# eric-downes/tianshou_marl

Hardware: AMD Instinct MI355X
Metric: env-steps/sec (n_env x n_agent) incl. PPO update, simple_spread N=3 (higher is better)
Workload: dtype f32; 1 GPU; simple_spread_v3 N=3 shared PPO, num_envs=1024 per GPU, obs 18, A=5, T=25, MLP 64-64; minibatch=4096, repeat=1, dispatch=per_agent, parallelism=env-shard x1

## Files before the change

### tianshou_marl_amd/csrc/mlp_tile.h

```cpp
#pragma once
#include "common.h"

namespace {

constexpr int R = 16;
constexpr int NT = 256;
constexpr int kMaxJ = 4;

struct Dims {
    int D, A;
    int Kp1;
    int nJ;
    int ld1;
};

__host__ __device__ constexpr Dims dims_const(int D, int A) {
    Dims d{};
    d.D = D; d.A = A; d.Kp1 = (D + 3) / 4 * 4; d.nJ = (D + 15) / 16; d.ld1 = 16 * ((D + 15) / 16) + 2;
    return d;
}

template <int H>
struct Lay {
    static constexpr int ldh = H + 2;
    static constexpr int ld2 = 2 * H + 2;
    static constexpr int ldo = 18;
    int W1, W2a, W2c, W3a, W3c, B1, B2, B3a, B3c, X, H1, H2, OUT, D3, D2, D1, total;
    __host__ __device__ Lay(const Dims &d, bool bwd) {
        int o = 0;
        W1 = o; o += 2 * H * d.ld1;
        W2a = o; o += H * ldh;
        W2c = o; o += H * ldh;
        W3a = o; o += 16 * ldh;
        W3c = o; o += H;
        B1 = o; o += 2 * H;
        B2 = o; o += 2 * H;
        B3a = o; o += 16;
        B3c = o; o += 2;
        o = (o + 3) & ~3;
        X = o; o += R * d.ld1;
        H1 = o; o += R * ld2;
        H2 = o; o += R * ld2;
        OUT = o; o += R * ldo;
        D3 = o; o += bwd ? R * ldo : 0;
        D2 = o; o += bwd ? R * ld2 : 0;
        D1 = o; o += bwd ? R * ld2 : 0;
        total = o;
    }
};

__device__ __forceinline__ f4 mfma(float a, float b, f4 c) {
    return __builtin_amdgcn_mfma_f32_16x16x4f32(a, b, c, 0, 0, 0);
}

template <int N>
__device__ __forceinline__ float fmaf_chain_ahead(const float *h, const float *w) {
    constexpr int Q = 8;
    static_assert(N % (2 * Q) == 0, "pairs of whole groups");
    float h0[Q], w0[Q], h1[Q], w1[Q], s = 0.f;
    int off = 0;
    auto pin = [&]() { asm volatile("" : "+v"(s), "+v"(off)); };
#pragma unroll
    for (int p = 0; p < Q; ++p) { h0[p] = h[p]; w0[p] = w[p]; }
#pragma unroll
    for (int j0 = 0; j0 < N; j0 += 2 * Q) {
        pin();
#pragma unroll
        for (int p = 0; p < Q; ++p) { h1[p] = h[off + j0 + Q + p]; w1[p] = w[off + j0 + Q + p]; }
#pragma unroll
        for (int p = 0; p < Q; ++p) s = fmaf(h0[p], w0[p], s);
        pin();
        if (j0 + 2 * Q < N) {
#pragma unroll
            for (int p = 0; p < Q; ++p) { h0[p] = h[off + j0 + 2 * Q + p]; w0[p] = w[off + j0 + 2 * Q + p]; }
        }
#pragma unroll
        for (int p = 0; p < Q; ++p) s = fmaf(h1[p], w1[p], s);
    }
    return s;
}

template <int H>
struct POff {
    int aW1, ab1, aW2, ab2, aW3, ab3, cW1, cb1, cW2, cb2, cW3, cb3, total;
    __host__ __device__ POff(int D, int A) {
        int o = 0;
        aW1 = o; o += H * D; ab1 = o; o += H; aW2 = o; o += H * H; ab2 = o; o += H; aW3 = o; o += A * H; ab3 = o; o += A;
        cW1 = o; o += H * D; cb1 = o; o += H; cW2 = o; o += H * H; cb2 = o; o += H; cW3 = o; o += H; cb3 = o; o += 1;
        total = o;
    }
};

template <int H>
__device__ void stage_weights(float *lds, const Lay<H> &ly, const Dims &d, const float *__restrict__ P, int tid_in = -1) {
    const POff<H> po(d.D, d.A);
    const int tid = tid_in < 0 ? (int)threadIdx.x : tid_in;
    constexpr int U = 12;
    for (int e0 = tid; e0 < 2 * H * d.ld1; e0 += U * NT) {
        float v[U];
#pragma unroll
        for (int u = 0; u < U; ++u) {
            const int e = e0 + u * NT;
            const int row = e / d.ld1, c = e - row * d.ld1;
            v[u] = 0.f;
            if (e < 2 * H * d.ld1 && c < d.D) v[u] = row < H ? P[po.aW1 + row * d.D + c] : P[po.cW1 + (row - H) * d.D + c];
        }
#pragma unroll
        for (int u = 0; u < U; ++u)
            if (e0 + u * NT < 2 * H * d.ld1) lds[ly.W1 + e0 + u * NT] = v[u];
    }
    for (int e0 = tid; e0 < H * ly.ldh; e0 += U * NT) {
        float va[U], vc[U];
#pragma unroll
        for (int u = 0; u < U; ++u) {
            const int e = e0 + u * NT;
            const int row = e / ly.ldh, c = e - row * ly.ldh;
            const bool on = e < H * ly.ldh && c < H;
            va[u] = on ? P[po.aW2 + row * H + c] : 0.f;
            vc[u] = on ? P[po.cW2 + row * H + c] : 0.f;
        }
#pragma unroll
        for (int u = 0; u < U; ++u) {
            const int e = e0 + u * NT;
            if (e < H * ly.ldh) { lds[ly.W2a + e] = va[u]; lds[ly.W2c + e] = vc[u]; }
        }
    }
    {
        constexpr int N3 = (16 * Lay<H>::ldh + NT - 1) / NT;
        float v3[N3], vv[5];
#pragma unroll
        for (int u = 0; u < N3; ++u) {
            const int e = tid + u * NT, row = e / ly.ldh, c = e - row * ly.ldh;
            v3[u] = (e < 16 * ly.ldh && row < d.A && c < H) ? P[po.aW3 + row * H + c] : 0.f;
        }
        const int e5 = tid < H ? tid : 0;
        vv[0] = P[po.cW3 + e5]; vv[1] = P[po.ab1 + e5]; vv[2] = P[po.cb1 + e5]; vv[3] = P[po.ab2 + e5]; vv[4] = P[po.cb2 + e5];
#pragma unroll
        for (int u = 0; u < N3; ++u) {
            const int e = tid + u * NT;
            if (e < 16 * ly.ldh) lds[ly.W3a + e] = v3[u];
        }
        if (tid < H) {
            lds[ly.W3c + tid] = vv[0]; lds[ly.B1 + tid] = vv[1]; lds[ly.B1 + H + tid] = vv[2]; lds[ly.B2 + tid] = vv[3];
            lds[ly.B2 + H + tid] = vv[4];
        }
    }
    if (tid < 16) lds[ly.B3a + tid] = tid < d.A ? P[po.ab3 + tid] : 0.f;
    if (tid == 0) lds[ly.B3c] = P[po.cb3];
}

constexpr int kStageChunk = 4 * 256;
__host__ __device__ inline int image_f4_padded(int x_floats) {
    return ((x_floats / 4) + kStageChunk - 1) / kStageChunk * kStageChunk;
}

template <int H>
__device__ __forceinline__ void stage_image(float *lds, const Lay<H> &ly, const float *__restrict__ img) {
    const int n4p = image_f4_padded(ly.X);
    const int wave_base = (threadIdx.x >> 6) * 64;
    for (int e = 0; e < n4p; e += NT) {
        __builtin_amdgcn_global_load_lds(
            (const __attribute__((address_space(1))) void *)(img + (size_t)(e + threadIdx.x) * 4),
            (__attribute__((address_space(3))) void *)(lds + (size_t)(e + wave_base) * 4), 16, 0, 0);
    }
}

template <int H>
__device__ __forceinline__ void tile_forward(float *lds, const Lay<H> &ly, const Dims &d) {
    const int lane = threadIdx.x & 63, w = threadIdx.x >> 6;
    const int r16 = lane & 15, kq = lane >> 4;
    {
        f4 acc_a = {0.f, 0.f, 0.f, 0.f}, acc_c = {0.f, 0.f, 0.f, 0.f};
        const float *xa = lds + ly.X + r16 * d.ld1 + kq;
        const float *wa = lds + ly.W1 + (16 * w + r16) * d.ld1 + kq;
        const float *wc = lds + ly.W1 + (H + 16 * w + r16) * d.ld1 + kq;
        for (int k0 = 0; k0 < d.Kp1; k0 += 4) {
            const float a = xa[k0];
            acc_a = mfma(a, wa[k0], acc_a);
            acc_c = mfma(a, wc[k0], acc_c);
        }
        const int col = 16 * w + r16;
        const float ba = lds[ly.B1 + col], bc = lds[ly.B1 + H + col];
#pragma unroll
        for (int r = 0; r < 4; ++r) {
            const int row = kq * 4 + r;
            lds[ly.H1 + row * ly.ld2 + col] = fmaxf(acc_a[r] + ba, 0.f);
            lds[ly.H1 + row * ly.ld2 + H + col] = fmaxf(acc_c[r] + bc, 0.f);
        }
    }
    __syncthreads();
    {
        f4 acc_a = {0.f, 0.f, 0.f, 0.f}, acc_c = {0.f, 0.f, 0.f, 0.f};
        const float *ha = lds + ly.H1 + r16 * ly.ld2 + kq;
        const float *hc = ha + H;
        const float *wa = lds + ly.W2a + (16 * w + r16) * ly.ldh + kq;
        const float *wc = lds + ly.W2c + (16 * w + r16) * ly.ldh + kq;
#pragma unroll
        for (int k0 = 0; k0 < H; k0 += 4) {
            acc_a = mfma(ha[k0], wa[k0], acc_a);
            acc_c = mfma(hc[k0], wc[k0], acc_c);
        }
        const int col = 16 * w + r16;
        const float ba = lds[ly.B2 + col], bc = lds[ly.B2 + H + col];
#pragma unroll
        for (int r = 0; r < 4; ++r) {
            const int row = kq * 4 + r;
            lds[ly.H2 + row * ly.ld2 + col] = fmaxf(acc_a[r] + ba, 0.f);
            lds[ly.H2 + row * ly.ld2 + H + col] = fmaxf(acc_c[r] + bc, 0.f);
        }
    }
    __syncthreads();
    if (w == 0) {
        f4 acc = {0.f, 0.f, 0.f, 0.f};
        const float *ha = lds + ly.H2 + r16 * ly.ld2 + kq;
        const float *wa = lds + ly.W3a + r16 * ly.ldh + kq;
#pragma unroll
        for (int k0 = 0; k0 < H; k0 += 4) acc = mfma(ha[k0], wa[k0], acc);
        const float b = lds[ly.B3a + r16];
#pragma unroll
        for (int r = 0; r < 4; ++r) lds[ly.OUT + (kq * 4 + r) * ly.ldo + r16] = acc[r] + b;
    } else if (w == 1 && lane < R) {
        const float *hc = lds + ly.H2 + lane * ly.ld2 + H;
        float s = 0.f;
        for (int j = 0; j < H; ++j) s = fmaf(hc[j], lds[ly.W3c + j], s);
        lds[ly.OUT + lane * ly.ldo + 16] = s + lds[ly.B3c];
    }
    __syncthreads();
}

template <int H>
__device__ __forceinline__ void tile_forward_split(float *lds, const Lay<H> &ly, const Dims &d) {
    const int lane = threadIdx.x & 63, w8 = threadIdx.x >> 6, net = w8 >> 2, w = w8 & 3;
    const int r16 = lane & 15, kq = lane >> 4;
    const int col = 16 * w + r16;
    {
        f4 acc = {0.f, 0.f, 0.f, 0.f};
        const float *xa = lds + ly.X + r16 * d.ld1 + kq;
        const float *wp = lds + ly.W1 + (net * H + col) * d.ld1 + kq;
        for (int k0 = 0; k0 < d.Kp1; k0 += 4) acc = mfma(xa[k0], wp[k0], acc);
        const float b = lds[ly.B1 + net * H + col];
#pragma unroll
        for (int r = 0; r < 4; ++r) lds[ly.H1 + (kq * 4 + r) * ly.ld2 + net * H + col] = fmaxf(acc[r] + b, 0.f);
    }
    __syncthreads();
    {
        f4 acc = {0.f, 0.f, 0.f, 0.f};
        const float *ha = lds + ly.H1 + r16 * ly.ld2 + net * H + kq;
        const float *wp = lds + (net ? ly.W2c : ly.W2a) + col * ly.ldh + kq;
#pragma unroll
        for (int k0 = 0; k0 < H; k0 += 4) acc = mfma(ha[k0], wp[k0], acc);
        const float b = lds[ly.B2 + net * H + col];
#pragma unroll
        for (int r = 0; r < 4; ++r) lds[ly.H2 + (kq * 4 + r) * ly.ld2 + net * H + col] = fmaxf(acc[r] + b, 0.f);
    }
    __syncthreads();
    if (w8 == 0) {
        f4 acc = {0.f, 0.f, 0.f, 0.f};
        const float *ha = lds + ly.H2 + r16 * ly.ld2 + kq;
        const float *wa = lds + ly.W3a + r16 * ly.ldh + kq;
#pragma unroll
        for (int k0 = 0; k0 < H; k0 += 4) acc = mfma(ha[k0], wa[k0], acc);
        const float b = lds[ly.B3a + r16];
#pragma unroll
        for (int r = 0; r < 4; ++r) lds[ly.OUT + (kq * 4 + r) * ly.ldo + r16] = acc[r] + b;
    } else if (w8 == 5 && lane < R) {
        const float *hc = lds + ly.H2 + lane * ly.ld2 + H;
        float s = 0.f;
        for (int j = 0; j < H; ++j) s = fmaf(hc[j], lds[ly.W3c + j], s);
        lds[ly.OUT + lane * ly.ldo + 16] = s + lds[ly.B3c];
    }
    __syncthreads();
}

constexpr int kXRegs = (R * (16 * kMaxJ + 2) + NT - 1) / NT;

template <int HAS_PERM = -1>
__device__ __forceinline__ void prefetch_tile_ids_load(int64_t (&id)[kXRegs + 1], const Dims &d, const int64_t *__restrict__ perm,
                                                       int64_t first, int64_t row0, int64_t M) {
    const int64_t ir = row0 + (threadIdx.x >> 4);
    if (HAS_PERM == 1 || (HAS_PERM == -1 && perm)) {
#pragma unroll
        for (int it = 0; it < kXRegs; ++it) {
            const int e = threadIdx.x + it * NT, r = e / d.ld1;
            const int64_t i = row0 + r;
            id[it] = perm[(e < R * d.ld1 && i < M) ? i : row0];
        }
        id[kXRegs] = perm[ir < M ? ir : row0];
    } else {
#pragma unroll
        for (int it = 0; it < kXRegs; ++it) id[it] = first + row0 + (threadIdx.x + it * NT) / d.ld1;
        id[kXRegs] = first + ir;
    }
}
__device__ __forceinline__ int64_t prefetch_tile_ids_done(int64_t (&xs)[kXRegs], const int64_t (&id)[kXRegs + 1], const Dims &d,
                                                          int64_t row0, int64_t M) {
#pragma unroll
    for (int it = 0; it < kXRegs; ++it) {
        const int e = threadIdx.x + it * NT, r = e / d.ld1, c = e - r * d.ld1;
        xs[it] = (e < R * d.ld1 && c < d.D && row0 + r < M) ? id[it] * d.D + c : -1;
    }
    return row0 + (threadIdx.x >> 4) < M ? id[kXRegs] : -1;
}
__device__ __forceinline__ int64_t prefetch_tile_ids_done_nb(int64_t (&xs)[kXRegs], unsigned &ok, const int64_t (&id)[kXRegs + 1],
                                                             const Dims &d, int64_t row0, int64_t M) {
    ok = 0;
#pragma unroll
    for (int it = 0; it < kXRegs; ++it) {
        const int e = threadIdx.x + it * NT, r = e / d.ld1, c = e - r * d.ld1;
        xs[it] = id[it] * d.D + (c < d.D ? c : 0);
        ok |= (unsigned)(e < R * d.ld1 && c < d.D && row0 + r < M) << it;
    }
    return row0 + (threadIdx.x >> 4) < M ? id[kXRegs] : -1;
}
__device__ __forceinline__ void prefetch_tile_vals_nb(float (&xr)[kXRegs], const int64_t (&xs)[kXRegs], unsigned ok,
                                                      const float *__restrict__ obs) {
#pragma unroll
    for (int it = 0; it < kXRegs; ++it) {
        const float v = obs[xs[it]];
        xr[it] = (ok >> it & 1u) ? v : 0.f;
    }
}
__device__ __forceinline__ void prefetch_tile_ids(int64_t (&xs)[kXRegs], const Dims &d,
                                                  const int64_t *__restrict__ perm, int64_t first, int64_t row0,
                                                  int64_t M) {
    int64_t id[kXRegs + 1];
    prefetch_tile_ids_load(id, d, perm, first, row0, M);
    (void)prefetch_tile_ids_done(xs, id, d, row0, M);
}

__device__ __forceinline__ void prefetch_tile_vals(float (&xr)[kXRegs], const int64_t (&xs)[kXRegs],
                                                   const float *__restrict__ obs) {
#pragma unroll
    for (int it = 0; it < kXRegs; ++it) {
        const float v = obs[xs[it] >= 0 ? xs[it] : 0];
        xr[it] = xs[it] >= 0 ? v : 0.f;
    }
}

__device__ __forceinline__ void prefetch_tile_x(float (&xr)[kXRegs], const Dims &d, const float *__restrict__ obs,
                                                const int64_t *__restrict__ perm, int64_t first, int64_t row0,
                                                int64_t M) {
    int64_t xs[kXRegs];
    prefetch_tile_ids(xs, d, perm, first, row0, M);
    prefetch_tile_vals(xr, xs, obs);
}

__device__ __forceinline__ void commit_tile_x(float *lds, int X, const Dims &d, const float (&xr)[kXRegs]) {
#pragma unroll
    for (int it = 0; it < kXRegs; ++it) {
        const int e = threadIdx.x + it * NT;
        if (e < R * d.ld1) lds[X + e] = xr[it];
    }
}

__device__ __forceinline__ void load_tile_x(float *lds, int X, const Dims &d, const float *__restrict__ obs,
                                            const int64_t *__restrict__ perm, int64_t first, int64_t row0,
                                            int64_t M) {
    float xr[kXRegs];
    prefetch_tile_x(xr, d, obs, perm, first, row0, M);
    commit_tile_x(lds, X, d, xr);
}

static int make_dims(int32_t obs_dim, int32_t hidden, int32_t n_act, Dims *d) {
    TSM_REQUIRE(hidden == 64, "fused MLP supports hidden == 64 (got %d)", hidden);
    TSM_REQUIRE(obs_dim >= 1 && obs_dim <= 16 * kMaxJ, "fused MLP supports 1 <= obs_dim <= %d (got %d)", 16 * kMaxJ,
                obs_dim);
    TSM_REQUIRE(n_act >= 1 && n_act <= 16, "fused MLP supports 1 <= n_act <= 16 (got %d)", n_act);
    d->D = obs_dim;
    d->A = n_act;
    d->Kp1 = (obs_dim + 3) / 4 * 4;
    d->nJ = (obs_dim + 15) / 16;
    d->ld1 = 16 * d->nJ + 2;
    return TSM_OK;
}


}
```

### tianshou_marl_amd/csrc/rollout.hip

```cpp
#include "common.h"
#include "mlp_tile.h"
#include "mpe_dev.h"
#include "philox.h"
#include "rollout_dev.h"
#include "wave_mlp.h"

int tsm_mpe_check_cfg(const tsm_mpe_cfg *h, MpeCfg *c);
extern long long *g_tsm_stamps;

namespace {

struct RolloutArgs {
    const float *P, *img;
    Dims d;
    uint64_t pol_seed, offset;
    const uint64_t *offset_dev;
    int mode;
    MpeCfg c;
    uint64_t env_seed;
    uint64_t *episode_ctr;
    float *apos, *avel, *lpos;
    int32_t *steps;
    int auto_reset;
    float *obs_cur_out;
    RolloutBufArgs b;
    long long *stamps;
};


#define XSTAMP(k) do { if (a.stamps && blockIdx.x == 0 && threadIdx.x == 0 && t < 4) a.stamps[900 + t * 8 + (k)] = (long long)wall_clock64(); } while (0)
#define STAMP(k) do { if (a.stamps && blockIdx.x == 0 && threadIdx.x == 0 && t < 4) a.stamps[t * 8 + (k)] = (long long)wall_clock64(); } while (0)

struct RtLay {
    int XN0, AP, AV, LP, REW, LOGP, VAL, MIN, ACT, STEPS, DONE, ROW, EP, CX, CY, CV, U, ANY, total;
    __host__ __device__ RtLay(int fwd_total, int ld1) {
        int o = fwd_total;
        XN0 = o; o += R * ld1;
        AP = o; o += R * 2;
        AV = o; o += R * 2;
        LP = o; o += R * 2;
        REW = o; o += R;
        LOGP = o; o += R;
        VAL = o; o += R;
        MIN = o; o += R;
        ACT = o; o += R;
        STEPS = o; o += R;
        DONE = o; o += 2 * R;
        o = (o + 1) & ~1;
        ROW = o; o += 2 * 2 * R;
        EP = o; o += 2 * R;
        o = (o + 3) & ~3;
        CX = o; o += R * 8;
        CY = o; o += R * 8;
        CV = o; o += R * 8;
        U = o; o += 2 * R;
        ANY = o; o += 2;
        o += 3 * R + 12;
        total = o;
    }
};

template <int H, int NT2, int DS = 0, int NS = 0>
__global__ __launch_bounds__(NT2) void rollout_kernel(RolloutArgs a) {
    extern __shared__ __attribute__((aligned(16))) float lds[];
    const Dims d = DS ? dims_const(DS, 5) : a.d;
    MpeCfg c_ = a.c;
    if (NS) { c_.N = NS; c_.obs_dim = DS; }
    const MpeCfg c = c_;
    const Lay<H> ly(d, false);
    const int N = c.N, D = d.D, st = 2 * N;
    const int EPB = R / N;
    const int e0 = blockIdx.x * EPB;
    const int n_here = min(EPB, c.n_env - e0);
    const int rows_here = n_here * N;
    const int64_t B = c.n_env;
    const RtLay tl(ly.total, d.ld1);
    float *XN0 = lds + tl.XN0, *s_ap = lds + tl.AP, *s_av = lds + tl.AV, *s_lp = lds + tl.LP, *s_rew = lds + tl.REW,
          *s_logp = lds + tl.LOGP, *s_val = lds + tl.VAL, *s_m = lds + tl.MIN, *s_cx = lds + tl.CX, *s_cy = lds + tl.CY, *s_u = lds + tl.U;
    int *s_act = reinterpret_cast<int *>(lds + tl.ACT), *s_steps = reinterpret_cast<int *>(lds + tl.STEPS),
        *s_done = reinterpret_cast<int *>(lds + tl.DONE), *s_cv = reinterpret_cast<int *>(lds + tl.CV),
        *s_any = reinterpret_cast<int *>(lds + tl.ANY);
    int64_t *s_row = reinterpret_cast<int64_t *>(lds + tl.ROW);
    uint64_t *s_ep = reinterpret_cast<uint64_t *>(lds + tl.EP);

    if (a.stamps && threadIdx.x == 0 && blockIdx.x < 256) a.stamps[64 + 2 * blockIdx.x] = (long long)wall_clock64();
    const bool main_t = threadIdx.x < NT;
    if (main_t) {
        if (a.img) stage_image<H>(lds, ly, a.img);
        else stage_weights<H>(lds, ly, d, a.P);
    }
    for (int i = threadIdx.x; i < R * d.ld1; i += NT2) { lds[ly.X + i] = 0.f; XN0[i] = 0.f; }
    const VrbState vs = vrb_view(a.b.vrb_state, B, N);
    const int r = threadIdx.x, el = r / N, ai = r - el * N;
    const bool lane_live = r < rows_here;
    const int e = e0 + el;
    constexpr int kEnvBase = NT2 >= 512 ? 256 : 64, kUBase = NT2 >= 512 ? 320 : 128;
    const int bel = (int)threadIdx.x - kEnvBase;
    const bool env_lane = bel >= 0 && bel < n_here;
    const int be = e0 + bel;
    constexpr bool DEFER = NT2 >= 512;
    constexpr int kRewBase = 384;
    const int wl = (int)threadIdx.x - kRewBase;
    const bool rew_lane = DEFER && wl >= 0 && wl < rows_here;
    constexpr int kRetBase = 448;
    const int rl = (int)threadIdx.x - kRetBase;
    const bool ret_lane = DEFER ? (rl >= 0 && rl < n_here) : env_lane;
    const int rq = DEFER ? rl : bel;
    bool pending = false;
    VrbLane vl;
    int n_fin_r = 0;
    EpReturns<kMpeMaxN> epr;
    if (ret_lane) epr.load(vs, N, e0 + rq);
    auto step_returns = [&](int tt, bool trq) {
        const int64_t bq = e0 + rq;
        const bool recq = trq && a.b.ep_rec && n_fin_r < a.b.max_ep;
        epr.fold(a.b.ep_rew_out, a.b.ep_rec, a.b.max_ep, N, B, bq, (int64_t)tt * B + bq, trq, recq, n_fin_r, s_rew + rq * N);
    };
    if (env_lane) {
        vl.load(vs, be);
        s_steps[bel] = a.steps[be];
        s_done[bel] = 1; s_done[R + bel] = 1;
        s_row[bel] = 0; s_row[R + bel] = 0;
    }
    for (int i = threadIdx.x; i < n_here * st; i += NT2) {
        s_ap[i] = a.apos[(int64_t)e0 * st + i];
        s_av[i] = a.avel[(int64_t)e0 * st + i];
        s_lp[i] = a.lpos[(int64_t)e0 * st + i];
    }
    const uint64_t off0 = a.offset + (a.offset_dev ? *a.offset_dev : 0ull);
    const int ur = (int)threadIdx.x - kUBase;
    const bool u_lane = a.mode == 1 && ur >= 0 && ur < rows_here;
    if (u_lane) s_u[ur] = tsm_philox_uniform(a.pol_seed, off0 + (uint64_t)e0 * N + (uint64_t)ur);
    __syncthreads();
    Lay<H> lyf = ly;
    int xcur = ly.X, xnxt = tl.XN0;
    for (int i = threadIdx.x; i < rows_here * D; i += NT2) {
        const int rr = i / D, k = i - rr * D, ee = rr / N;
        lds[xcur + rr * d.ld1 + k] = mpe_obs_elem(c, s_ap + ee * st, s_av + ee * st, s_lp + ee * st, rr - ee * N, k);
    }
    __syncthreads();

    for (int t = 0; t <= a.b.n_steps; ++t) {
        const int g = (t & 1) * R;
        const bool last = t == a.b.n_steps;
        float *XN = lds + xnxt;
        STAMP(0);
        if (a.stamps && blockIdx.x == 0 && threadIdx.x == 0 && t < 64) a.stamps[640 + t] = (long long)wall_clock64();
        STAMP(1);
        lyf.X = xcur;
        if constexpr (NT2 == 2 * NT) tile_forward_split<H>(lds, lyf, d);
        else tile_forward<H>(lds, lyf, d);
        STAMP(2);
        bool tr = false;
        if (env_lane && !last) {
            const int stp = s_steps[bel] + 1;
            tr = stp >= c.max_cycles;
            s_steps[bel] = stp;
            const VrbStep sp = vl.add(vs, a.b.S, t, be, B, tr, a.b.done_store, a.b.ptr_out, a.b.ep_len_out, a.b.ep_idx_out, a.b.ep_rec, a.b.max_ep);
            vl.n_fin += tr ? 1 : 0;
            s_row[g + bel] = sp.row;
            s_done[g + bel] = tr ? 1 : 0;
            const unsigned long long ends = __ballot(tr);
            if (bel == 0) s_any[t & 1] = ends != 0ull;
        }
        if (u_lane && !last) s_u[((t + 1) & 1) * R + ur] = tsm_philox_uniform(a.pol_seed, off0 + (uint64_t)(t + 1) * B * N + (uint64_t)e0 * N + (uint64_t)ur);
        if (DEFER && pending) {
            if (wl >= 0 && wl < 64) {
                const int wr = wl < rows_here ? wl : 0;
                const int wel = wr / N, wai = wr - wel * N;
                const int64_t rowq = s_row[(g ^ R) + wel];
                const MpePos pos = mpe_load_pos(c, s_ap + wel * st);
                const float md = mpe_landmark_min_dist(c, pos, s_lp + wel * st, wai);
                const float local = mpe_local_penalty(c, pos, s_ap + wel * st, wai);
                float mv[kMpeMaxN];
#pragma unroll
                for (int l = 0; l < kMpeMaxN; ++l) mv[l] = l < N ? __shfl(md, wel * N + l, 64) : 0.f;
                const float rw = mpe_reward_regs(c, mv, local);
                if (wl < rows_here) { s_rew[wl] = rw; a.b.rew_store[rowq * N + wai] = rw; }
            }
            pending = false;
        }
        auto pair_task = [&](int p) {
            const int rp = p >> 3, jp = p & 7;
            float sx = 0.f, sy = 0.f;
            int ok = 0;
            if (rp < rows_here && jp < N) {
                const int ep = rp / N, ip = rp - ep * N;
                const float *ap = s_ap + ep * st;
                if (jp != ip) ok = mpe_pair_force(c, ap[2 * ip], ap[2 * ip + 1], ap[2 * jp], ap[2 * jp + 1], ip, jp, sx, sy) ? 1 : 0;
            }
            s_cx[p] = sx; s_cy[p] = sy; s_cv[p] = ok;
        };
        if (DEFER && !last) {
            if (N <= 4) { if (rl >= 0 && rl < 64) pair_task(((rl >> 2) << 3) | (rl & 3)); }
            else if (rl >= 0 && rl < 64) pair_task(rl);
            else if (ur >= 0 && ur < 64) pair_task(64 + ur);
        }
        if (main_t) {
            const int hr = threadIdx.x >> 4, j = threadIdx.x & 15;
            const float *lg = lds + ly.OUT + hr * ly.ldo;
            const bool on = j < d.A;
            const float x = on ? lg[j] : -INFINITY;
            const float m = row16_max(x);
            const float ex = on ? expf(x - m) : 0.f;
            const int gbase = threadIdx.x & 48;
            float ssum = 0.f;
            row_prefix_sum<0>(ex, d.A, ssum);
            if (j == 0 && hr < rows_here) {
                const float val = lg[16];
                const int hel = hr / N;
                if (!s_done[(g ^ R) + hel] && a.b.vnext_store)
                    a.b.vnext_store[s_row[(g ^ R) + hel] * N + (hr - hel * N)] = val;
                if (!last) s_val[hr] = val;
            }
            if (!last) {
                int act = 0;
                if (a.mode == 1) {
                    const float u = s_u[(t & 1) * R + (hr < rows_here ? hr : 0)] * ssum;
                    float cs = 0.f;
                    act = d.A - 1;
                    bool found = false;
                    row_cdf_pick<0>(ex, d.A, u, cs, act, found);
                } else {
                    const unsigned long long eq = __ballot(on && x == m);
                    act = __ffsll((long long)((eq >> gbase) & 0xFFFFull)) - 1;
                }
                const float la = __shfl(x, gbase + act, 64);
                if (j == 0 && hr < rows_here) {
                    s_act[hr] = act;
                    s_logp[hr] = la - (m + logf(ssum));
                }
            }
        }
        __syncthreads();
        STAMP(3);
        if (DEFER && t > 0 && ret_lane) {
            step_returns(t - 1, s_done[(g ^ R) + rq] != 0);
        }
        if (last) {
            if (a.obs_cur_out)
                for (int i = threadIdx.x; i < rows_here * D; i += NT2) {
                    const int rr = i / D, k = i - rr * D;
                    a.obs_cur_out[((int64_t)e0 * N + rr) * D + k] = lds[xcur + rr * d.ld1 + k];
                }
            break;
        }
        if constexpr (!DEFER) {
            if (threadIdx.x < R * 8) pair_task(threadIdx.x);
            XSTAMP(5);
            __syncthreads();
        }
        XSTAMP(0);
        if (lane_live) {
            const float px = s_ap[el * st + 2 * ai], py = s_ap[el * st + 2 * ai + 1];
            const float vx = s_av[el * st + 2 * ai], vy = s_av[el * st + 2 * ai + 1];
            float fx = mpe_action_force(c, s_act[r], 0);
            float fy = mpe_action_force(c, s_act[r], 1);
            mpe_pair_fold(c, s_cx, s_cy, s_cv, r, fx, fy);
            float npx, npy, nvx, nvy;
            mpe_integrate(c, px, py, vx, vy, fx, fy, npx, npy, nvx, nvy);
            s_ap[el * st + 2 * ai] = npx; s_ap[el * st + 2 * ai + 1] = npy;
            s_av[el * st + 2 * ai] = nvx; s_av[el * st + 2 * ai + 1] = nvy;
        }
        __syncthreads();
        XSTAMP(1);
        const int any_done = s_any[t & 1];
        const bool now = !DEFER || any_done;
        if (now) {
            float local = 0.f;
            if (lane_live) {
                const MpePos pos = mpe_load_pos(c, s_ap + el * st);
                s_m[r] = mpe_landmark_min_dist(c, pos, s_lp + el * st, ai);
                local = mpe_local_penalty(c, pos, s_ap + el * st, ai);
            }
            XSTAMP(2);
            if (!DEFER && threadIdx.x >= 64)
                for (int i = threadIdx.x - 64; i < rows_here * D; i += NT2 - 64) {
                    const int rr = i / D, k = i - rr * D, ee = rr / N;
                    XN[rr * d.ld1 + k] =
                        mpe_obs_elem(c, s_ap + ee * st, s_av + ee * st, s_lp + ee * st, rr - ee * N, k);
                }
            __syncthreads();
            XSTAMP(3);
            if (lane_live) s_rew[r] = mpe_reward(c, s_m + el * N, local);
            __syncthreads();
            XSTAMP(4);
            if (!DEFER && ret_lane) {
                step_returns(t, s_done[g + rq] != 0);
            }
        }
        STAMP(4);
        for (int i = threadIdx.x; i < rows_here * D; i += NT2) {
            const int rr = i / D, k = i - rr * D, ee = rr / N;
            float v;
            if constexpr (DEFER) {
                v = mpe_obs_elem(c, s_ap + ee * st, s_av + ee * st, s_lp + ee * st, rr - ee * N, k);
                XN[rr * d.ld1 + k] = v;
            } else {
                v = XN[rr * d.ld1 + k];
            }
            const int64_t dst = (s_row[g + ee] * N + (rr - ee * N)) * D + k;
            a.b.obs_store[dst] = lds[xcur + rr * d.ld1 + k];
            if (a.b.obs_next_store) a.b.obs_next_store[dst] = v;
        }
        if (ur >= 0 && ur < rows_here) {
            const int pel = ur / N, pai = ur - pel * N;
            const int64_t dst = s_row[g + pel] * N + pai;
            a.b.act_store[dst] = s_act[ur];
            if (now) a.b.rew_store[dst] = s_rew[ur];
            a.b.term_store[dst] = 0;
            a.b.trunc_store[dst] = (uint8_t)s_done[g + pel];
            if (a.b.logp_store) a.b.logp_store[dst] = s_logp[ur];
            if (a.b.vs_store) a.b.vs_store[dst] = s_val[ur];
        }
        if constexpr (DEFER) __syncthreads();
        pending = !now;
        STAMP(5);
        if (any_done) {
            if (a.b.vnext_store) {
                lyf.X = xnxt;
                if constexpr (NT2 == 2 * NT) tile_forward_split<H>(lds, lyf, d);
                else tile_forward<H>(lds, lyf, d);
                if (lane_live && s_done[g + el]) a.b.vnext_store[s_row[g + el] * N + ai] = lds[ly.OUT + r * ly.ldo + 16];
            }
            if (a.auto_reset) {
                if (env_lane && s_done[g + bel]) {
                    const uint64_t ep = a.episode_ctr[be];
                    s_ep[bel] = ep;
                    a.episode_ctr[be] = ep + 1;
                    s_steps[bel] = 0;
                }
                __syncthreads();
                if (lane_live && s_done[g + el])
                    mpe_reset_agent(c, e, a.env_seed, s_ep[el], ai, s_ap + el * st, s_av + el * st, s_lp + el * st);
                __syncthreads();
                for (int i = threadIdx.x; i < rows_here * D; i += NT2) {
                    const int rr = i / D, k = i - rr * D, ee = rr / N;
                    if (s_done[g + ee])
                        XN[rr * d.ld1 + k] =
                            mpe_obs_elem(c, s_ap + ee * st, s_av + ee * st, s_lp + ee * st, rr - ee * N, k);
                }
                __syncthreads();
            }
        }
        { const int tmp = xcur; xcur = xnxt; xnxt = tmp; }
        STAMP(6);
    }
    __syncthreads();
    if (a.stamps && threadIdx.x == 0 && blockIdx.x < 256) a.stamps[65 + 2 * blockIdx.x] = (long long)wall_clock64();
    for (int i = threadIdx.x; i < n_here * st; i += NT2) {
        a.apos[(int64_t)e0 * st + i] = s_ap[i];
        a.avel[(int64_t)e0 * st + i] = s_av[i];
        a.lpos[(int64_t)e0 * st + i] = s_lp[i];
    }
    if (env_lane) {
        a.steps[be] = s_steps[bel];
        vl.store(vs, a.b.ep_rec, be);
    }
    if (ret_lane) epr.store(vs, N, e0 + rq);
    rollout_advance_counter(a.b.done_ctr, a.b.offset_dev_rw, a.b.offset_inc, threadIdx.x == 0);
}

struct Rw64Lay {
    static constexpr int kLdc = 68;
    int AP, AV, LP, LG, H2C, VAL, CX, CY, CV, MIN, REW, LOGP, ACT, STEPS, DONE, ROW, EP, size;
    __host__ __device__ Rw64Lay() {
        int q = 0;
        AP = q; q += 2 * R;
        AV = q; q += 2 * R;
        LP = q; q += 2 * R;
        LG = q; q += R * 16;
        H2C = q; q += R * kLdc;
        VAL = q; q += R;
        CX = q; q += R * 8;
        CY = q; q += R * 8;
        CV = q; q += R * 8;
        MIN = q; q += R;
        REW = q; q += R;
        LOGP = q; q += R;
        ACT = q; q += R;
        STEPS = q; q += R;
        DONE = q; q += R;
        ROW = q; q += 2 * R;
        EP = q; q += 2 * R;
        size = (q + 3) & ~3;
    }
};

template <int NJ, int DS = 0, int NS = 0>
__global__ __launch_bounds__(NT) void rollout_wave64_kernel(RolloutArgs a) {
    constexpr int H = 64, MB = H / 16, KB1 = 4 * NJ, KBH = H / 4;
    extern __shared__ __attribute__((aligned(16))) float lds[];
    const Dims d = DS ? dims_const(DS, 5) : a.d;
    MpeCfg c_ = a.c;
    if (NS) { c_.N = NS; c_.obs_dim = DS; }
    const MpeCfg c = c_;
    const Lay<H> ly(d, false);
    const Rw64Lay wl;
    constexpr int ld1 = 16 * NJ + 2;
    const int tid = threadIdx.x, lane = tid & 63, w = tid >> 6, n_waves = blockDim.x >> 6, c16 = lane & 15, kq = lane >> 4;
    const int N = c.N, D = d.D, A = d.A, st = 2 * N;
    const int EPW = R / N;
    const int e0 = (blockIdx.x * n_waves + w) * EPW;
    const int n_here = max(0, min(EPW, c.n_env - e0));
    const int rows_here = n_here * N;
    const int64_t B = c.n_env;
    const int img_floats = image_f4_padded(ly.X) * 4;
    if (a.img) {
        const int n4p = img_floats / 4, wave_base = w * 64;
        for (int e = 0; e < n4p; e += blockDim.x)
            __builtin_amdgcn_global_load_lds((const __attribute__((address_space(1))) void *)(a.img + (size_t)(e + tid) * 4),
                                             (__attribute__((address_space(3))) void *)(lds + (size_t)(e + wave_base) * 4), 16, 0, 0);
    } else {
        for (int v = tid; v < NT; v += blockDim.x) stage_weights<H>(lds, ly, d, a.P, v);
    }
    const int wvo = img_floats + w * wl.size;
    float *wv = lds + wvo;
    float *s_ap = wv + wl.AP, *s_av = wv + wl.AV, *s_lp = wv + wl.LP, *s_lg = wv + wl.LG, *s_h2c = wv + wl.H2C, *s_val = wv + wl.VAL,
          *s_cx = wv + wl.CX, *s_cy = wv + wl.CY, *s_m = wv + wl.MIN, *s_rew = wv + wl.REW, *s_logp = wv + wl.LOGP;
    int *s_cv = reinterpret_cast<int *>(wv + wl.CV), *s_act = reinterpret_cast<int *>(wv + wl.ACT),
        *s_steps = reinterpret_cast<int *>(wv + wl.STEPS), *s_done = reinterpret_cast<int *>(wv + wl.DONE);
    int64_t *s_row = reinterpret_cast<int64_t *>(wv + wl.ROW);
    uint64_t *s_ep = reinterpret_cast<uint64_t *>(wv + wl.EP);

    const VrbState vs = vrb_view(a.b.vrb_state, B, N);
    const int r = lane, el = r / N, ai = r - el * N;
    const bool lane_live = r < rows_here;
    const int e = e0 + el;
    const int bel = lane - 16;
    const bool env_lane = bel >= 0 && bel < n_here;
    const int be = e0 + bel;
    VrbLane vl;
    EpReturns<kMpeMaxN> epr;
    if (env_lane) {
        vl.load(vs, be);
        epr.load(vs, N, be);
    }
    float st_ap = 0.f, st_av = 0.f, st_lp = 0.f;
    if (lane < n_here * st) {
        st_ap = a.apos[(int64_t)e0 * st + lane]; st_av = a.avel[(int64_t)e0 * st + lane]; st_lp = a.lpos[(int64_t)e0 * st + lane];
    }
    const int steps0 = env_lane ? a.steps[be] : 0;
    const uint64_t off0 = a.offset + (a.offset_dev ? *a.offset_dev : 0ull);
    __syncthreads();
    if (n_here == 0) return;
    if (env_lane) { s_steps[bel] = steps0; s_done[bel] = 1; s_row[bel] = 0; }
    if (lane < n_here * st) { s_ap[lane] = st_ap; s_av[lane] = st_av; s_lp[lane] = st_lp; }
    if (lane < 16) s_lg[16 * 16 - 1 - lane] = 0.f;

    const int zoff = wvo + wl.LG + 16 * 15 + 15;
    uint32_t el_ab[KB1];
    const int sn_el = c16 / N, sn_ai = c16 - sn_el * N;
    const bool sn_live = c16 < rows_here;
#pragma unroll
    for (int kb = 0; kb < KB1; ++kb) {
        const int k = 4 * kb + kq;
        const int base = wvo + sn_el * st;
        el_ab[kb] = sn_live && k < D ? mpe_obs_offsets(N, base + wl.AP, base + wl.AV, base + wl.LP, zoff, sn_ai, k) : mpe_obs_offsets_zero(zoff);
    }
    const int ND = N * D;
    const int obs_col = sn_ai * D + kq;
    int pair_ei[2];
#pragma unroll
    for (int q = 0; q < 2; ++q) {
        const int rp = (lane + 64 * q) >> 3, ep = rp / N;
        pair_ei[q] = rp < rows_here ? (ep << 3) | (rp - ep * N) : -1;
    }
    const int kb1_n = d.Kp1 >> 2;
    const float *w1a = lds + ly.W1 + c16 * ld1 + kq, *w1c = w1a + H * ld1;
    const float *w2a = lds + ly.W2a + c16 * ly.ldh + kq, *w2c = lds + ly.W2c + c16 * ly.ldh + kq, *w3a = lds + ly.W3a + c16 * ly.ldh + kq;
    auto critic_value = [&](const float (&x)[KB1]) -> float {
        f4 acc[MB];
        float hb[4 * MB];
        wave_layer<MB, KB1>(w1c, ld1, x, kb1_n, acc);
        wave_bias_relu<MB, true>(lds + ly.B1 + H + 4 * kq, acc);
        wave_to_frags<MB>(acc, hb);
        wave_layer<MB, KBH>(w2c, ly.ldh, hb, KBH, acc);
        wave_bias_relu<MB, true>(lds + ly.B2 + H + 4 * kq, acc);
#pragma unroll
        for (int mb = 0; mb < MB; ++mb) *reinterpret_cast<f4 *>(s_h2c + c16 * Rw64Lay::kLdc + 16 * mb + 4 * kq) = acc[mb];
        float s = 0.f;
        if (lane < R) {
            f4 hv[H / 4], wq[H / 4];
#pragma unroll
            for (int q = 0; q < H / 4; ++q) {
                hv[q] = *reinterpret_cast<const f4 *>(s_h2c + lane * Rw64Lay::kLdc + 4 * q);
                wq[q] = *reinterpret_cast<const f4 *>(lds + ly.W3c + 4 * q);
            }
#pragma unroll
            for (int j = 0; j < H; ++j) s = fmaf(hv[j >> 2][j & 3], wq[j >> 2][j & 3], s);
            s += lds[ly.B3c];
        }
        return s;
    };

    for (int t = 0; t <= a.b.n_steps; ++t) {
        const bool last = t == a.b.n_steps;
        int64_t p_row = 0;
        int p_done = 1;
        if (lane_live) { p_row = s_row[el]; p_done = s_done[el]; }
        bool tr = false, rec = false;
        int64_t o = 0;
        if (env_lane && !last) {
            const int stp = s_steps[bel] + 1;
            tr = stp >= c.max_cycles;
            s_steps[bel] = stp;
            const VrbStep sp = vl.add(vs, a.b.S, t, be, B, tr, a.b.done_store, a.b.ptr_out, a.b.ep_len_out, a.b.ep_idx_out, a.b.ep_rec, a.b.max_ep);
            o = sp.o; rec = sp.rec;
            s_row[bel] = sp.row;
            s_done[bel] = tr ? 1 : 0;
        }
        float xb[KB1];
        wave_obs_frags(lds, el_ab, xb);
        if (last) {
            if (a.obs_cur_out && sn_live) wave_obs_rows_out(a.obs_cur_out + ((int64_t)e0 * N + c16) * D + kq, xb, D, kq);
        } else if (sn_live) {
            wave_obs_rows_out(a.b.obs_store + s_row[sn_el] * ND + obs_col, xb, D, kq);
        }
        const float val = critic_value(xb);
        if (lane_live && !p_done && a.b.vnext_store) a.b.vnext_store[p_row * N + ai] = val;
        if (last) break;
        {
            f4 acc[MB];
            float hb[4 * MB];
            wave_layer<MB, KB1>(w1a, ld1, xb, kb1_n, acc);
            wave_bias_relu<MB, true>(lds + ly.B1 + 4 * kq, acc);
            wave_to_frags<MB>(acc, hb);
            wave_layer<MB, KBH>(w2a, ly.ldh, hb, KBH, acc);
            wave_bias_relu<MB, true>(lds + ly.B2 + 4 * kq, acc);
            wave_to_frags<MB>(acc, hb);
            f4 lg = f4{0.f, 0.f, 0.f, 0.f};
#pragma unroll
            for (int kb = 0; kb < KBH; ++kb) lg = wave_mfma4(w3a[4 * kb], hb[kb], lg);
            const f4 b = *reinterpret_cast<const f4 *>(lds + ly.B3a + 4 * kq);
            if (!(c16 == 15 && kq == 3))
                *reinterpret_cast<f4 *>(s_lg + c16 * 16 + 4 * kq) = f4{lg[0] + b[0], lg[1] + b[1], lg[2] + b[2], lg[3] + b[3]};
        }
        if (lane_live) {
            float lgv[8], ex[8];
            {
                const f4 l0 = *reinterpret_cast<const f4 *>(s_lg + lane * 16), l1 = *reinterpret_cast<const f4 *>(s_lg + lane * 16 + 4);
                lgv[0] = l0[0]; lgv[1] = l0[1]; lgv[2] = l0[2]; lgv[3] = l0[3]; lgv[4] = l1[0]; lgv[5] = l1[1]; lgv[6] = l1[2]; lgv[7] = l1[3];
            }
            float m = -INFINITY;
            int arg = 0;
#pragma unroll
            for (int j = 0; j < 8; ++j) if (j < A && lgv[j] > m) { m = lgv[j]; arg = j; }
            float s = 0.f;
#pragma unroll
            for (int j = 0; j < 8; ++j) { ex[j] = 0.f; if (j < A) { ex[j] = expf(lgv[j] - m); s += ex[j]; } }
            const float lse = m + logf(s);
            int act = arg;
            if (a.mode == 1) {
                const uint64_t gi = (uint64_t)e0 * N + (uint64_t)lane;
                const float u = tsm_philox_uniform(a.pol_seed, off0 + (uint64_t)t * B * N + gi) * s;
                float cs = 0.f;
                bool found = false;
                act = A - 1;
#pragma unroll
                for (int j = 0; j < 8; ++j)
                    if (j < A) {
                        cs += ex[j];
                        if (!found && u < cs) { act = j; found = true; }
                    }
            }
            float la = lgv[0];
#pragma unroll
            for (int j = 1; j < 8; ++j) la = act == j ? lgv[j] : la;
            s_act[lane] = act;
            s_logp[lane] = la - lse;
            s_val[lane] = val;
        }
        mpe_pair_tasks(c, pair_ei, lane, 64, s_ap, s_cx, s_cy, s_cv);
        if (lane_live) {
            const float px = s_ap[el * st + 2 * ai], py = s_ap[el * st + 2 * ai + 1];
            const float vx = s_av[el * st + 2 * ai], vy = s_av[el * st + 2 * ai + 1];
            float fx = mpe_action_force(c, s_act[r], 0);
            float fy = mpe_action_force(c, s_act[r], 1);
            mpe_pair_fold(c, s_cx, s_cy, s_cv, r, fx, fy);
            float npx, npy, nvx, nvy;
            mpe_integrate(c, px, py, vx, vy, fx, fy, npx, npy, nvx, nvy);
            s_ap[el * st + 2 * ai] = npx; s_ap[el * st + 2 * ai + 1] = npy;
            s_av[el * st + 2 * ai] = nvx; s_av[el * st + 2 * ai + 1] = nvy;
        }
        float local = 0.f;
        if (lane_live) {
            const MpePos pos = mpe_load_pos(c, s_ap + el * st);
            s_m[r] = mpe_landmark_min_dist(c, pos, s_lp + el * st, ai);
            local = mpe_local_penalty(c, pos, s_ap + el * st, ai);
        }
        float xn[KB1];
        const unsigned long long done_mask = __ballot(lane_live && s_done[el]);
        if (a.b.obs_next_store || (done_mask && a.b.vnext_store)) wave_obs_frags(lds, el_ab, xn);
        if (a.b.obs_next_store && sn_live) wave_obs_rows_out(a.b.obs_next_store + s_row[sn_el] * ND + obs_col, xn, D, kq);
        if (lane_live) {
            float mv[kMpeMaxN];
#pragma unroll
            for (int l = 0; l < kMpeMaxN; ++l) mv[l] = s_m[el * N + (l < N ? l : N - 1)];
            float global = 0.f;
#pragma unroll
            for (int l = 0; l < kMpeMaxN; ++l) if (l < N) global -= mv[l];
            s_rew[r] = global * (1.f - c.local_ratio) + local * c.local_ratio;
        }
        if (env_lane) epr.fold(a.b.ep_rew_out, a.b.ep_rec, a.b.max_ep, N, B, be, o, tr, rec, vl.n_fin, s_rew + bel * N);
        if (lane_live) {
            const int64_t dst = s_row[el] * N + ai;
            a.b.act_store[dst] = s_act[r];
            a.b.rew_store[dst] = s_rew[r];
            a.b.term_store[dst] = 0;
            a.b.trunc_store[dst] = (uint8_t)s_done[el];
            if (a.b.logp_store) a.b.logp_store[dst] = s_logp[r];
            if (a.b.vs_store) a.b.vs_store[dst] = s_val[r];
        }
        if (done_mask) {
            if (a.b.vnext_store) {
                const float vt = critic_value(xn);
                if (lane_live && s_done[el]) a.b.vnext_store[s_row[el] * N + ai] = vt;
            }
            if (a.auto_reset) {
                if (env_lane && s_done[bel]) {
                    const uint64_t ep = a.episode_ctr[be];
                    s_ep[bel] = ep;
                    a.episode_ctr[be] = ep + 1;
                    s_steps[bel] = 0;
                }
                if (lane_live && s_done[el])
                    mpe_reset_agent(c, e, a.env_seed, s_ep[el], ai, s_ap + el * st, s_av + el * st, s_lp + el * st);
            }
        }
    }
    if (lane < n_here * st) {
        a.apos[(int64_t)e0 * st + lane] = s_ap[lane];
        a.avel[(int64_t)e0 * st + lane] = s_av[lane];
        a.lpos[(int64_t)e0 * st + lane] = s_lp[lane];
    }
    if (env_lane) {
        a.steps[be] = s_steps[bel];
        vl.store(vs, a.b.ep_rec, be);
        epr.store(vs, N, be);
    }
    rollout_advance_counter(a.b.done_ctr, a.b.offset_dev_rw, a.b.offset_inc, tid == 0);
}

__global__ void u64_add_kernel(uint64_t *p, uint64_t inc) { *p += inc; }

}

TSM_EXPORT int tsm_u64_add(uint64_t *counter, uint64_t inc, void *stream) {
    TSM_REQUIRE(counter, "tsm_u64_add: null pointer");
    hipLaunchKernelGGL(u64_add_kernel, dim3(1), dim3(1), 0, tsm_stream(stream), counter, inc);
    TSM_LAUNCH_CHECK();
    return TSM_OK;
}

TSM_EXPORT int tsm_rollout_spread(const tsm_rollout_desc *desc_host, void *stream) {
    TSM_REQUIRE(desc_host, "tsm_rollout_spread: null descriptor");
    const tsm_rollout_desc &h = *desc_host;
    RolloutArgs a;
    if (int rc = make_dims(h.obs_dim, h.hidden, h.n_act, &a.d)) return rc;
    if (int rc = tsm_mpe_check_cfg(&h.env, &a.c)) return rc;
    TSM_REQUIRE(a.c.obs_dim == h.obs_dim, "tsm_rollout_spread: obs_dim %d != 6 * n_agent", h.obs_dim);
// ... 71 lines not shown
```

Measured before the change: 167.6 million env-steps/s.

## Overlap weight staging with state loads and restructure rollout epilogue

Weight staging becomes two phases. All threads first issue the global weight loads into registers, then the env state, step counts and offset loads are issued, and only afterwards do the weights go to LDS. The aim is to overlap load latency in the prologue. The extra t == n_steps iteration is removed from the main loop. In its place is a dedicated epilogue that writes the state back, runs a bootstrap forward pass only when some env continues, and flushes the pending rewards and returns. This cuts per-step `last` branching and may skip the final forward pass. In exchange it raises register pressure from the staged weights and duplicates some epilogue logic, so it risks subtle ordering or sync differences.

```diff
diff --git a/tianshou_marl_amd/csrc/mlp_tile.h b/tianshou_marl_amd/csrc/mlp_tile.h
--- a/tianshou_marl_amd/csrc/mlp_tile.h
+++ b/tianshou_marl_amd/csrc/mlp_tile.h
@@ -149,6 +149,63 @@
     if (tid == 0) lds[ly.B3c] = P[po.cb3];
 }
 
+template <int H, int NTH>
+struct StagedWeights {
+    static constexpr int K1 = (2 * H * (16 * kMaxJ + 2) + NTH - 1) / NTH, K2 = (H * Lay<H>::ldh + NTH - 1) / NTH,
+                         K3 = (16 * Lay<H>::ldh + NTH - 1) / NTH;
+    float w1[K1], w2a[K2], w2c[K2], w3[K3], vv[5], b3a, b3c;
+
+    __device__ __forceinline__ void issue(const Dims &d, const float *__restrict__ P) {
+        const POff<H> po(d.D, d.A);
+        const int tid = threadIdx.x;
+        constexpr int ldh = Lay<H>::ldh;
+#pragma unroll
+        for (int u = 0; u < K1; ++u) {
+            const int e = tid + u * NTH, row = e / d.ld1, c = e - row * d.ld1;
+            w1[u] = 0.f;
+            if (e < 2 * H * d.ld1 && c < d.D) w1[u] = row < H ? P[po.aW1 + row * d.D + c] : P[po.cW1 + (row - H) * d.D + c];
+        }
+#pragma unroll
+        for (int u = 0; u < K2; ++u) {
+            const int e = tid + u * NTH, row = e / ldh, c = e - row * ldh;
+            const bool on = e < H * ldh && c < H;
+            w2a[u] = on ? P[po.aW2 + row * H + c] : 0.f;
+            w2c[u] = on ? P[po.cW2 + row * H + c] : 0.f;
+        }
+#pragma unroll
+        for (int u = 0; u < K3; ++u) {
+            const int e = tid + u * NTH, row = e / ldh, c = e - row * ldh;
+            w3[u] = (e < 16 * ldh && row < d.A && c < H) ? P[po.aW3 + row * H + c] : 0.f;
+        }
+        const int e5 = tid < H ? tid : 0;
+        vv[0] = P[po.cW3 + e5]; vv[1] = P[po.ab1 + e5]; vv[2] = P[po.cb1 + e5]; vv[3] = P[po.ab2 + e5]; vv[4] = P[po.cb2 + e5];
+        b3a = tid < d.A ? P[po.ab3 + tid] : 0.f;
+        b3c = tid == 0 ? P[po.cb3] : 0.f;
+    }
+
+    __device__ __forceinline__ void commit(float *lds, const Lay<H> &ly, const Dims &d) const {
+        const int tid = threadIdx.x;
+        constexpr int ldh = Lay<H>::ldh;
+#pragma unroll
+        for (int u = 0; u < K1; ++u)
+            if (tid + u * NTH < 2 * H * d.ld1) lds[ly.W1 + tid + u * NTH] = w1[u];
+#pragma unroll
+        for (int u = 0; u < K2; ++u) {
+            const int e = tid + u * NTH;
+            if (e < H * ldh) { lds[ly.W2a + e] = w2a[u]; lds[ly.W2c + e] = w2c[u]; }
+        }
+#pragma unroll
+        for (int u = 0; u < K3; ++u)
+            if (tid + u * NTH < 16 * ldh) lds[ly.W3a + tid + u * NTH] = w3[u];
+        if (tid < H) {
+            lds[ly.W3c + tid] = vv[0]; lds[ly.B1 + tid] = vv[1]; lds[ly.B1 + H + tid] = vv[2]; lds[ly.B2 + tid] = vv[3];
+            lds[ly.B2 + H + tid] = vv[4];
+        }
+        if (tid < 16) lds[ly.B3a + tid] = b3a;
+        if (tid == 0) lds[ly.B3c] = b3c;
+    }
+};
+
 constexpr int kStageChunk = 4 * 256;
 __host__ __device__ inline int image_f4_padded(int x_floats) {
     return ((x_floats / 4) + kStageChunk - 1) / kStageChunk * kStageChunk;
diff --git a/tianshou_marl_amd/csrc/rollout.hip b/tianshou_marl_amd/csrc/rollout.hip
--- a/tianshou_marl_amd/csrc/rollout.hip
+++ b/tianshou_marl_amd/csrc/rollout.hip
@@ -32,7 +32,7 @@
 #define STAMP(k) do { if (a.stamps && blockIdx.x == 0 && threadIdx.x == 0 && t < 4) a.stamps[t * 8 + (k)] = (long long)wall_clock64(); } while (0)
 
 struct RtLay {
-    int XN0, AP, AV, LP, REW, LOGP, VAL, MIN, ACT, STEPS, DONE, ROW, EP, CX, CY, CV, U, ANY, total;
+    int XN0, AP, AV, LP, REW, LOGP, VAL, MIN, ACT, STEPS, DONE, ROW, EP, CX, CY, CV, U, ANY, BOOT, total;
     __host__ __device__ RtLay(int fwd_total, int ld1) {
         int o = fwd_total;
         XN0 = o; o += R * ld1;
@@ -55,6 +55,7 @@
         CV = o; o += R * 8;
         U = o; o += 2 * R;
         ANY = o; o += 2;
+        BOOT = o;
         o += 3 * R + 12;
         total = o;
     }
@@ -79,17 +80,16 @@
           *s_logp = lds + tl.LOGP, *s_val = lds + tl.VAL, *s_m = lds + tl.MIN, *s_cx = lds + tl.CX, *s_cy = lds + tl.CY, *s_u = lds + tl.U;
     int *s_act = reinterpret_cast<int *>(lds + tl.ACT), *s_steps = reinterpret_cast<int *>(lds + tl.STEPS),
         *s_done = reinterpret_cast<int *>(lds + tl.DONE), *s_cv = reinterpret_cast<int *>(lds + tl.CV),
-        *s_any = reinterpret_cast<int *>(lds + tl.ANY);
+        *s_any = reinterpret_cast<int *>(lds + tl.ANY), *s_boot = reinterpret_cast<int *>(lds + tl.BOOT);
     int64_t *s_row = reinterpret_cast<int64_t *>(lds + tl.ROW);
     uint64_t *s_ep = reinterpret_cast<uint64_t *>(lds + tl.EP);
 
     if (a.stamps && threadIdx.x == 0 && blockIdx.x < 256) a.stamps[64 + 2 * blockIdx.x] = (long long)wall_clock64();
     const bool main_t = threadIdx.x < NT;
-    if (main_t) {
-        if (a.img) stage_image<H>(lds, ly, a.img);
-        else stage_weights<H>(lds, ly, d, a.P);
-    }
-    for (int i = threadIdx.x; i < R * d.ld1; i += NT2) { lds[ly.X + i] = 0.f; XN0[i] = 0.f; }
+    const uint64_t off_dev = a.offset_dev ? *a.offset_dev : 0ull;
+    StagedWeights<H, NT2> sw;
+    if (a.img) { if (main_t) stage_image<H>(lds, ly, a.img); }
+    else sw.issue(d, a.P);
     const VrbState vs = vrb_view(a.b.vrb_state, B, N);
     const int r = threadIdx.x, el = r / N, ai = r - el * N;
     const bool lane_live = r < rows_here;
@@ -116,21 +116,30 @@
         const bool recq = trq && a.b.ep_rec && n_fin_r < a.b.max_ep;
         epr.fold(a.b.ep_rew_out, a.b.ep_rec, a.b.max_ep, N, B, bq, (int64_t)tt * B + bq, trq, recq, n_fin_r, s_rew + rq * N);
     };
+    int steps0 = 0;
     if (env_lane) {
         vl.load(vs, be);
-        s_steps[bel] = a.steps[be];
+        steps0 = a.steps[be];
+    }
+    const bool st_lane = (int)threadIdx.x < n_here * st;
+    float st_ap = 0.f, st_av = 0.f, st_lp = 0.f;
+    if (st_lane) {
+        st_ap = a.apos[(int64_t)e0 * st + threadIdx.x];
+        st_av = a.avel[(int64_t)e0 * st + threadIdx.x];
+        st_lp = a.lpos[(int64_t)e0 * st + threadIdx.x];
+    }
+    for (int i = threadIdx.x; i < R * d.ld1; i += NT2) { lds[ly.X + i] = 0.f; XN0[i] = 0.f; }
+    if (env_lane) {
         s_done[bel] = 1; s_done[R + bel] = 1;
         s_row[bel] = 0; s_row[R + bel] = 0;
     }
-    for (int i = threadIdx.x; i < n_here * st; i += NT2) {
-        s_ap[i] = a.apos[(int64_t)e0 * st + i];
-        s_av[i] = a.avel[(int64_t)e0 * st + i];
-        s_lp[i] = a.lpos[(int64_t)e0 * st + i];
-    }
-    const uint64_t off0 = a.offset + (a.offset_dev ? *a.offset_dev : 0ull);
+    const uint64_t off0 = a.offset + off_dev;
     const int ur = (int)threadIdx.x - kUBase;
     const bool u_lane = a.mode == 1 && ur >= 0 && ur < rows_here;
     if (u_lane) s_u[ur] = tsm_philox_uniform(a.pol_seed, off0 + (uint64_t)e0 * N + (uint64_t)ur);
+    if (!a.img) sw.commit(lds, ly, d);
+    if (env_lane) s_steps[bel] = steps0;
+    if (st_lane) { s_ap[threadIdx.x] = st_ap; s_av[threadIdx.x] = st_av; s_lp[threadIdx.x] = st_lp; }
     __syncthreads();
     Lay<H> lyf = ly;
     int xcur = ly.X, xnxt = tl.XN0;
@@ -140,9 +149,24 @@
     }
     __syncthreads();
 
-    for (int t = 0; t <= a.b.n_steps; ++t) {
+    auto late_rewards = [&](int gp) {
+        if (wl >= 0 && wl < 64) {
+            const int wr = wl < rows_here ? wl : 0;
+            const int wel = wr / N, wai = wr - wel * N;
+            const int64_t rowq = s_row[gp + wel];
+            const MpePos pos = mpe_load_pos(c, s_ap + wel * st);
+            const float md = mpe_landmark_min_dist(c, pos, s_lp + wel * st, wai);
+            const float local = mpe_local_penalty(c, pos, s_ap + wel * st, wai);
+            float mv[kMpeMaxN];
+#pragma unroll
+            for (int l = 0; l < kMpeMaxN; ++l) mv[l] = l < N ? __shfl(md, wel * N + l, 64) : 0.f;
+            const float rw = mpe_reward_regs(c, mv, local);
+            if (wl < rows_here) { s_rew[wl] = rw; a.b.rew_store[rowq * N + wai] = rw; }
+        }
+    };
+
+    for (int t = 0; t < a.b.n_steps; ++t) {
         const int g = (t & 1) * R;
-        const bool last = t == a.b.n_steps;
         float *XN = lds + xnxt;
         STAMP(0);
         if (a.stamps && blockIdx.x == 0 && threadIdx.x == 0 && t < 64) a.stamps[640 + t] = (long long)wall_clock64();
@@ -152,7 +176,7 @@
         else tile_forward<H>(lds, lyf, d);
         STAMP(2);
         bool tr = false;
-        if (env_lane && !last) {
+        if (env_lane) {
             const int stp = s_steps[bel] + 1;
             tr = stp >= c.max_cycles;
             s_steps[bel] = stp;
@@ -161,23 +185,12 @@
             s_row[g + bel] = sp.row;
             s_done[g + bel] = tr ? 1 : 0;
             const unsigned long long ends = __ballot(tr);
-            if (bel == 0) s_any[t & 1] = ends != 0ull;
-        }
-        if (u_lane && !last) s_u[((t + 1) & 1) * R + ur] = tsm_philox_uniform(a.pol_seed, off0 + (uint64_t)(t + 1) * B * N + (uint64_t)e0 * N + (uint64_t)ur);
+            const unsigned long long goes_on = __ballot(!tr);
+            if (bel == 0) { s_any[t & 1] = ends != 0ull; s_boot[0] = goes_on != 0ull; }
+        }
+        if (u_lane) s_u[((t + 1) & 1) * R + ur] = tsm_philox_uniform(a.pol_seed, off0 + (uint64_t)(t + 1) * B * N + (uint64_t)e0 * N + (uint64_t)ur);
         if (DEFER && pending) {
-            if (wl >= 0 && wl < 64) {
-                const int wr = wl < rows_here ? wl : 0;
-                const int wel = wr / N, wai = wr - wel * N;
-                const int64_t rowq = s_row[(g ^ R) + wel];
-                const MpePos pos = mpe_load_pos(c, s_ap + wel * st);
-                const float md = mpe_landmark_min_dist(c, pos, s_lp + wel * st, wai);
-                const float local = mpe_local_penalty(c, pos, s_ap + wel * st, wai);
-                float mv[kMpeMaxN];
-#pragma unroll
-                for (int l = 0; l < kMpeMaxN; ++l) mv[l] = l < N ? __shfl(md, wel * N + l, 64) : 0.f;
-                const float rw = mpe_reward_regs(c, mv, local);
-                if (wl < rows_here) { s_rew[wl] = rw; a.b.rew_store[rowq * N + wai] = rw; }
-            }
+            late_rewards(g ^ R);
             pending = false;
         }
         auto pair_task = [&](int p) {
@@ -191,7 +204,7 @@
             }
             s_cx[p] = sx; s_cy[p] = sy; s_cv[p] = ok;
         };
-        if (DEFER && !last) {
+        if (DEFER) {
             if (N <= 4) { if (rl >= 0 && rl < 64) pair_task(((rl >> 2) << 3) | (rl & 3)); }
             else if (rl >= 0 && rl < 64) pair_task(rl);
             else if (ur >= 0 && ur < 64) pair_task(64 + ur);
@@ -211,9 +224,9 @@
                 const int hel = hr / N;
                 if (!s_done[(g ^ R) + hel] && a.b.vnext_store)
                     a.b.vnext_store[s_row[(g ^ R) + hel] * N + (hr - hel * N)] = val;
-                if (!last) s_val[hr] = val;
-            }
-            if (!last) {
+                s_val[hr] = val;
+            }
+            {
                 int act = 0;
                 if (a.mode == 1) {
                     const float u = s_u[(t & 1) * R + (hr < rows_here ? hr : 0)] * ssum;
@@ -236,14 +249,6 @@
         STAMP(3);
         if (DEFER && t > 0 && ret_lane) {
             step_returns(t - 1, s_done[(g ^ R) + rq] != 0);
-        }
-        if (last) {
-            if (a.obs_cur_out)
-                for (int i = threadIdx.x; i < rows_here * D; i += NT2) {
-                    const int rr = i / D, k = i - rr * D;
-                    a.obs_cur_out[((int64_t)e0 * N + rr) * D + k] = lds[xcur + rr * d.ld1 + k];
-                }
-            break;
         }
         if constexpr (!DEFER) {
             if (threadIdx.x < R * 8) pair_task(threadIdx.x);
@@ -346,17 +351,38 @@
         { const int tmp = xcur; xcur = xnxt; xnxt = tmp; }
         STAMP(6);
     }
-    __syncthreads();
+    {
+        const int gp = ((a.b.n_steps & 1) * R) ^ R;
+        if (a.stamps && blockIdx.x == 0 && threadIdx.x == 0 && a.b.n_steps < 64) a.stamps[640 + a.b.n_steps] = (long long)wall_clock64();
+        if (st_lane) {
+            a.apos[(int64_t)e0 * st + threadIdx.x] = s_ap[threadIdx.x];
+            a.avel[(int64_t)e0 * st + threadIdx.x] = s_av[threadIdx.x];
+            a.lpos[(int64_t)e0 * st + threadIdx.x] = s_lp[threadIdx.x];
+        }
+        if (env_lane) {
+            a.steps[be] = s_steps[bel];
+            vl.store(vs, a.b.ep_rec, be);
+        }
+        if (a.obs_cur_out)
+            for (int i = threadIdx.x; i < rows_here * D; i += NT2) {
+                const int rr = i / D, k = i - rr * D;
+                a.obs_cur_out[((int64_t)e0 * N + rr) * D + k] = lds[xcur + rr * d.ld1 + k];
+            }
+        const bool boot = a.b.vnext_store && s_boot[0];
+        if (boot) {
+            lyf.X = xcur;
+            if constexpr (NT2 == 2 * NT) tile_forward_split<H>(lds, lyf, d);
+            else tile_forward<H>(lds, lyf, d);
+            const int hr = threadIdx.x >> 4, hel = hr / N;
+            if (main_t && (threadIdx.x & 15) == 0 && hr < rows_here && !s_done[gp + hel])
+                a.b.vnext_store[s_row[gp + hel] * N + (hr - hel * N)] = lds[ly.OUT + hr * ly.ldo + 16];
+        }
+        if (DEFER) {
+            if (pending) { late_rewards(gp); __syncthreads(); }
+            if (ret_lane) step_returns(a.b.n_steps - 1, s_done[gp + rq] != 0);
+        }
+    }
     if (a.stamps && threadIdx.x == 0 && blockIdx.x < 256) a.stamps[65 + 2 * blockIdx.x] = (long long)wall_clock64();
-    for (int i = threadIdx.x; i < n_here * st; i += NT2) {
-        a.apos[(int64_t)e0 * st + i] = s_ap[i];
-        a.avel[(int64_t)e0 * st + i] = s_av[i];
-        a.lpos[(int64_t)e0 * st + i] = s_lp[i];
-    }
-    if (env_lane) {
-        a.steps[be] = s_steps[bel];
-        vl.store(vs, a.b.ep_rec, be);
-    }
     if (ret_lane) epr.store(vs, N, e0 + rq);
     rollout_advance_counter(a.b.done_ctr, a.b.offset_dev_rw, a.b.offset_inc, threadIdx.x == 0);
 }
```

After: 168.5 million env-steps/s (median of 6 runs). Within noise of the previous version (+0.5%).
